# kaleo996/F5E-TTS

Hardware: AMD Instinct MI355X
Metric: mel_frames_per_sec (higher is better)
Workload: dtype bf16; 1 GPU; C2: F5TTS_v1_Base random-init, batch 1 per GPU, N_ref=188 N=469 frames, euler NFE=32, CFG=2.0 (cond+uncond batched), sway=-1.0, hipGraph ODE loop, HIP log-mel front-end + Vocos decode on GPU; parallelism=replica x1 (utterance sharding, no collective on the data path)

## Files before the change

### f5e-tts_amd/_C.py

```python
from __future__ import annotations

import ctypes as C
import os

_HERE = os.path.dirname(os.path.abspath(__file__))
LIB_PATH = os.environ.get("F5E_HIP_LIB") or os.path.join(_HERE, "libf5e_hip.so")

ABI_VERSION = 2

ACT_NONE, ACT_SILU, ACT_GELU_ERF, ACT_GELU_TANH, ACT_RELU, ACT_MISH = range(6)

_P, _I, _F, _LL = C.c_void_p, C.c_int, C.c_float, C.c_longlong

SIGNATURES = {
    "f5e_abi_version": [],
    "f5e_last_error": [],
    "f5e_check_device": [],
    "f5e_gemm_bf16_bias": [_P, _P, _I, _P, _I, _P, _P, _I, _I, _I, _I, _I, _I, _I],
    "f5e_gemm_bf16_gate_residual": [_P, _P, _I, _P, _I, _P, _P, _I, _P, _I, _I, _P, _I, _I, _P, _I, _I, _I, _I],
    "f5e_gemm_bf16_qkv_rope": [_P, _P, _I, _P, _I, _P, _P, _P, _P, _I, _I, _I, _P, _P, _P, _I, _I, _I, _I],
    "f5e_gemm_bf16_bias_ln": [_P, _P, _I, _P, _I, _P, _P, _I, _I, _I, _I, _I, _I, _I, _P],
    "f5e_gemm_bf16_gate_residual_ln": [_P, _P, _I, _P, _I, _P, _P, _I, _P, _I, _I, _P, _I, _I, _P, _I, _I, _I, _I, _P],
    "f5e_gemm_bf16_qkv_rope_ln": [_P, _P, _I, _P, _I, _P, _P, _P, _P, _I, _I, _I, _P, _P, _P, _I, _I, _I, _I, _P],
    "f5e_adaln_pre": [_P, _P, _I, _P, _I, _P, _I, _I, _I, _P, _I, _P, _I, _P, _I, _I],
    "f5e_flash_attn": [_P, _P, _P, _P, _P, _I, _P, _I, _I, _I, _I, _I],
    "f5e_joint_attn": [_P, _P, _P, _P, _P, _P, _P, _P, _I, _P, _I, _P, _I, _I, _I, _I, _I, _I, _I],
    "f5e_layernorm": [_P, _P, _I, _P, _I, _I, _P, _P, _P, _P, _I, _I, _I, _P, _I, _I, _I, _F],
    "f5e_grn": [_P, _P, _P, _P, _P, _P, _I, _I, _I],
    "f5e_l2norm": [_P, _P, _I, _P, _I, _I, _P, _I, _I],
    "f5e_gemm_f32": [_P, _P, _I, _I, _I, _P, _I, _P, _I, _P, _P, _I, _I, _P, _P, _I, _P, _I, _I, _I, _I],
    "f5e_convpos": [_P, _P, _I, _P, _P, _I, _P, _I, _P, _I, _P, _I, _I, _I, _I, _I],
    "f5e_dwconv7": [_P, _P, _P, _P, _P, _I, _I, _I],
    "f5e_im2col": [_P, _P, _P, _I, _I, _I, _I, _I],
    "f5e_sinus_embed": [_P, _P, _P, _P, _I, _I, _F],
    "f5e_rope_table": [_P, _P, _P, _I, _I],
    "f5e_text_gather": [_P, _P, _P, _P, _P, _P, _I, _I, _I, _I, _I],
    "f5e_ode_update": [_P, _P, _LL, _I, _F, _F, _P, _P, _P, _P, _P, _P, _LL],
    "f5e_ode_update_traj": [_P, _P, _LL, _I, _F, _F, _P, _P, _P, _LL, _I, _P, _P, _P, _LL],
    "f5e_advance_eval": [_P, _P],
    "f5e_stitch": [_P, _P, _P, _P, _P, _LL, _I],
    "f5e_cast_bf16": [_P, _P, _P, _LL],
    "f5e_cast_f32": [_P, _P, _P, _LL],
    "f5e_axpby": [_P, _P, _P, _P, _F, _F, _F, _LL],
    "f5e_vq_eval": [_P, _P, _I, _P, _I, _P, _P, _P, _I, _I, _I, _I],
    "f5e_mas_workspace_bytes": [_I, _I, _I, C.POINTER(C.c_ulonglong)],
    "f5e_mas_path": [_P, _P, _LL, _I, _P, _P, _P, _P, _P, C.c_ulonglong, _I, _I, _I],
    "f5e_resample": [_P, _P, _LL, _P, _I, _I, _I, _P, _LL, _I, _I, _I],
    "f5e_ctc_align_workspace_bytes": [_I, _I, _I, C.POINTER(C.c_ulonglong)],
    "f5e_ctc_align": [_P, _P, _LL, _I, _P, _I, _P, _P, _I, _P, _P, _P, _P, _P, C.c_ulonglong, _I, _I, _I, _I],
    "f5e_ctc_greedy": [_P, _P, _LL, _I, _P, _I, _I, _P, _P, _P, _I, _I, _I],
    "f5e_ctc_beam_workspace_bytes": [_I, _I, _I, C.POINTER(C.c_ulonglong)],
    "f5e_ctc_beam": [_P, _P, _LL, _I, _P, _I, _I, _P, _I, _P, _P, _P, C.c_ulonglong, _I, _I, _I],
    "f5e_token_logp": [_P, _P, _LL, _P, _P, _LL, _I],
    "f5e_log_softmax_rows": [_P, _P, _LL, _P, _LL, _LL, _I],
    "f5e_stft_logmel": [_P, _P, _I, _I, _P, _P, _P, _P, _I, _I, _I, _I],
    "f5e_stft_logmel_banded": [_P, _P, _I, _I, _P, _P, _P, _P, _I, _P, _I, _I, _I, _I],
    "f5e_stft_logmel_banded_ex": [_P, _P, _I, _I, _P, _P, _P, _P, _I, _P, _I, _I, _I, _I, _I, _I, _F],
    "f5e_bigvgan_act": [_P, _P, _P, _I, _P, _P, _P, _P, _I, _I, _I],
    "f5e_bigvgan_conv": [_P, _P, _P, _P, _P, _P, _P, _F, _I, _I, _I, _I, _I, _I, _I, _I, _I],
    "f5e_bigvgan_post": [_P, _P, _P, _P, _P, _I, _I, _I, _I, _I],
    "f5e_istft_head": [_P, _P, _I, _P, _P, _P, _P, _I, _I, _I, _I],
    "f5e_kaldi_fbank": [_P, _P, _I, _I, _P, _P, _P, _P, _I, _I, _I, _I, _F, _F, _F],
    "f5e_glu": [_P, _P, _I, _P, _I, _LL, _I],
    "f5e_dwconv": [_P, _P, _P, _P, _P, _P, _I, _I, _I, _I],
    "f5e_softmax_rows": [_P, _P, _I, _P, _I, _P, _LL, _I, _I, _F],
    "f5e_dwconv_stream": [_P, _P, _P, _P, _P, _P, _I, _I, _I, _I, _I, _I],
    "f5e_relpos_attn": [_P, _P, _I, _P, _I, _P, _I, _P, _I, _P, _I, _P, _I, _I, _I, _I, _I, _I, _I, _F],
    "f5e_mha_f32": [_P, _P, _I, _P, _I, _P, _I, _P, _I, _P, _I, _I, _I, _I, _I, _I, _F],
    "f5e_attn_decode_f32": [_P, _P, _I, _P, _P, _LL, _I, _P, _I, _P, _I, _I, _I, _I, _I, _I, _F],
    "f5e_beam_step": [_P, _P, _LL, _P, _P, _P, _P, _P, _I, _P, _P, _P, _I, _I, _I, _I, _I],
    "f5e_dit_forward": [_P, _P],
    "f5e_sample_loop": [_P, _P],
    "f5e_workspace_bytes": [_P, _P],
    "f5e_timer_create": [_I, C.POINTER(C.c_void_p)],
    "f5e_timer_destroy": [_P],
    "f5e_timer_reset": [_P],
    "f5e_timer_read": [_P, C.POINTER(C.c_float), _I, C.POINTER(C.c_int)],
    "f5e_timer_read_ops": [_P, C.POINTER(C.c_int), _I, C.POINTER(C.c_int)],
    "f5e_graph_begin": [_P],
    "f5e_graph_end": [_P, C.POINTER(C.c_void_p)],
    "f5e_graph_launch": [_P, _P],
    "f5e_graph_destroy": [_P],
}
_RESTYPE = {"f5e_last_error": C.c_char_p}
# ... 76 lines not shown
```

### f5e-tts_amd/csrc/conv.hip

```cpp
#include <cstdlib>
#include "f5e_common.h"

namespace {

struct ConvPosArgs {
  const bf16* x; int ldx;
  const bf16* w;
  const float* bias;
  bf16* out_bf16; int ldo;
  float* out_f32; int ldo32;
  const float* resid; int ldr;
  int S, N, D, mode, tiles_t, cpg;
  unsigned long long* trace;
};

__device__ __forceinline__ void glds16c(const void* g, void* lds) {
  __builtin_amdgcn_global_load_lds((const __attribute__((address_space(1))) void*)g,
                                   (__attribute__((address_space(3))) void*)lds, 16, 0, 0);
}

__device__ const uint4 conv_zero16 = {0u, 0u, 0u, 0u};

__device__ __forceinline__ void wait_vm_lgkm0(int n) {
  switch (n) {
// ... 253 lines not shown
      for (int i = 0; i < 4; ++i)
#pragma unroll
        for (int j = 0; j < 4; ++j)
          acc[i][j] = __builtin_amdgcn_mfma_f32_16x16x32_bf16(wf[i], xf[j], acc[i][j], 0, 0, 0);
    };
    if (live) reads(0);
    if (u + NST - 1 < 8) stage_w((u + NST - 1) % NST, u + NST - 1);
    if (!live) break;
    mfmas();
    reads(1);
    mfmas();
  }

  if constexpr (TRC) ts[5] = __builtin_amdgcn_s_memtime();
  asm volatile("s_waitcnt vmcnt(0) lgkmcnt(0)" ::: "memory");
  __builtin_amdgcn_s_barrier();
  float* mine = Red + wave * (64 * RS);
#pragma unroll
  for (int i = 0; i < 4; ++i)
#pragma unroll
    for (int j = 0; j < 4; ++j) *(f32x4*)(mine + (j * 16 + fr) * RS + i * 16 + fq * 4) = acc[i][j];
  asm volatile("s_waitcnt lgkmcnt(0)" ::: "memory");
  __builtin_amdgcn_s_barrier();
#pragma unroll
  for (int p = 0; p < 4; ++p) asm volatile("" : "+v"(rv[p]));

  if (oc < a.cpg) {
#pragma unroll
    for (int p = 0; p < 4; ++p) {
      const int row = wave * 16 + p * 4 + (lane >> 4);
      const int t = t0 + row;
      const size_t m = (size_t)seq * a.N + t;
      const float* rp = Red + row * RS + oc;
      f32x4 v = (*(const f32x4*)rp + *(const f32x4*)(rp + 64 * RS)) + (*(const f32x4*)(rp + 2 * 64 * RS) + *(const f32x4*)(rp + 3 * 64 * RS));
      v += bias;
      v[0] = mish_f(v[0]); v[1] = mish_f(v[1]); v[2] = mish_f(v[2]); v[3] = mish_f(v[3]);
      if (t >= a.N) continue;
      if (a.mode == 0) {
        *(bf16x4*)(a.out_bf16 + m * a.ldo + n) = f2bf4(v[0], v[1], v[2], v[3]);
      } else {
        v += rv[p];
        *(f32x4*)(a.out_f32 + m * a.ldo32 + n) = v;
      }
    }
  }
  if constexpr (TRC) {
    asm volatile("s_waitcnt vmcnt(0)" ::: "memory");
    ts[6] = __builtin_amdgcn_s_memtime(); ts[7] = __builtin_amdgcn_s_memrealtime();
    if (tid == 0 && a.trace) {
      unsigned long long* o = a.trace + ((size_t)(blockIdx.z * gridDim.y + blockIdx.y) * gridDim.x + blockIdx.x) * 8;
#pragma unroll
      for (int i = 0; i < 8; ++i) o[i] = ts[i];
    }
  }
}

__global__ __launch_bounds__(256) void dwconv7_kernel(const float* x, const float* wT, const float* bias, float* y,
                                                       int B, int T, int C) {
  const int c4n = C / 4;
  const size_t total = (size_t)B * T * c4n;
  for (size_t i = (size_t)blockIdx.x * 256 + threadIdx.x; i < total; i += (size_t)gridDim.x * 256) {
    const int c = (int)(i % c4n) * 4;
    const size_t bt = i / c4n;
    const int t = (int)(bt % T);
    const size_t b = bt / T;
    f32x4 acc = *(const f32x4*)(bias + c);
#pragma unroll
    for (int j = 0; j < 7; ++j) {
      const int tj = t + j - 3;
      if (tj >= 0 && tj < T)
        acc += *(const f32x4*)(wT + (size_t)j * C + c) * *(const f32x4*)(x + (b * T + tj) * C + c);
    }
    *(f32x4*)(y + (b * T + t) * C + c) = acc;
  }
}

__global__ __launch_bounds__(256) void im2col_kernel(const float* x, float* col, int B, int T, int Cin, int ksize,
                                                      int pad) {
  const size_t total = (size_t)B * T * ksize * Cin;
  for (size_t i = (size_t)blockIdx.x * 256 + threadIdx.x; i < total; i += (size_t)gridDim.x * 256) {
    const int ic = (int)(i % Cin);
    size_t r = i / Cin;
    const int j = (int)(r % ksize);
    r /= ksize;
    const int t = (int)(r % T);
    const size_t b = r / T;
    const int tj = t + j - pad;
    col[i] = (tj >= 0 && tj < T) ? x[(b * T + tj) * Cin + ic] : 0.f;
  }
}

inline int grid_for(size_t total) {
  size_t g = (total + 255) / 256;
  return (int)(g < 4096 ? (g ? g : 1) : 4096);
}

}

#ifdef F5E_TOOLS
static unsigned long long* g_convpos_trace = nullptr;
#define F5E_CONVPOS_TRACE g_convpos_trace
#else
#define F5E_CONVPOS_TRACE ((unsigned long long*)nullptr)
#endif

extern "C" {
// ... 8 lines not shown
  F5E_REQUIRE(x && w_packed && bias, "convpos: null operand");
  F5E_REQUIRE(S > 0 && N > 0 && D > 0 && groups > 0 && D % groups == 0, "convpos: bad D=%d / groups=%d", D, groups);
  const int cpg = D / groups;
  F5E_REQUIRE(cpg % 16 == 0 && cpg <= 64, "convpos: channels per group = %d must be 16, 32, 48 or 64", cpg);
  F5E_REQUIRE(ldx % 8 == 0, "convpos: ldx must be a multiple of 8");
  if (mode == 0) F5E_REQUIRE(out_bf16 && ldo % 4 == 0, "convpos: mode 0 needs a bf16 output");
  else {
    F5E_REQUIRE(mode == 1, "convpos: mode must be 0 or 1");
    F5E_REQUIRE(out_f32 && resid && ldo32 % 4 == 0 && ldr % 4 == 0, "convpos: mode 1 needs f32 output + residual");
  }
  ConvPosArgs a{};
  a.x = (const bf16*)x; a.ldx = ldx; a.w = (const bf16*)w_packed; a.bias = bias;
  a.out_bf16 = (bf16*)out_bf16; a.ldo = ldo; a.out_f32 = out_f32; a.ldo32 = ldo32; a.resid = resid; a.ldr = ldr;
  a.S = S; a.N = N; a.D = D; a.mode = mode; a.cpg = cpg;
  a.tiles_t = (N + 63) / 64;
  F5E_REQUIRE(a.tiles_t <= 65535 && S <= 65535, "convpos: grid too large");
  const dim3 grid(groups, a.tiles_t, S);
  const int xs = 96 * 128;
#ifdef F5E_TOOLS
  static const int forced = getenv("F5E_CONVPOS") ? atoi(getenv("F5E_CONVPOS")) : 0;
#else
  constexpr int forced = 0;
#endif
  const int n_cu = f5e_cu_count();
  const bool split = forced ? forced == 1 : (size_t)groups * a.tiles_t * S <= (size_t)n_cu;
  const int lds_split = xs + 4 * 4 * 8192, lds_ring = xs + 4 * 8192;
  a.trace = F5E_CONVPOS_TRACE;
  static F5eDeviceOnce once_split;
  if (split) F5E_OPT_IN_LDS(once_split, convpos_split_kernel<false>, lds_split);
#ifdef F5E_TOOLS
  static F5eDeviceOnce once_split_trace;
  if (split && a.trace) {
    F5E_OPT_IN_LDS(once_split_trace, convpos_split_kernel<true>, lds_split);
    hipLaunchKernelGGL(convpos_split_kernel<true>, grid, dim3(256), lds_split, st, a);
  } else if (a.trace) {
    hipLaunchKernelGGL((convpos_kernel<4, true>), grid, dim3(256), lds_ring, st, a);
  } else
#endif
  if (split) {
    hipLaunchKernelGGL(convpos_split_kernel<false>, grid, dim3(256), lds_split, st, a);
  } else {
    hipLaunchKernelGGL((convpos_kernel<4, false>), grid, dim3(256), lds_ring, st, a);
  }
  F5E_LAUNCH_CHECK("convpos");
  return F5E_OK;
}

int f5e_convpos(hipStream_t st, const void* x, int ldx, const void* w_packed, const float* bias, int mode,
                void* out_bf16, int ldo, float* out_f32, int ldo32, const float* resid, int ldr, int S, int N, int D,
                int groups) {
  return convpos_launch(st, x, ldx, w_packed, bias, mode, out_bf16, ldo, out_f32, ldo32, resid, ldr, S, N, D, groups);
}

int f5e_dwconv7(hipStream_t st, const float* x, const float* w_t, const float* bias, float* y, int B, int T, int C) {
  F5E_REQUIRE(x && w_t && bias && y, "dwconv7: null operand");
  F5E_REQUIRE(B > 0 && T > 0 && C > 0 && C % 4 == 0, "dwconv7: C=%d must be a positive multiple of 4", C);
  hipLaunchKernelGGL(dwconv7_kernel, dim3(grid_for((size_t)B * T * C / 4)), dim3(256), 0, st, x, w_t, bias, y, B, T, C);
  F5E_LAUNCH_CHECK("dwconv7");
  return F5E_OK;
}

int f5e_im2col(hipStream_t st, const float* x, float* col, int B, int T, int Cin, int ksize, int pad) {
  F5E_REQUIRE(x && col && B > 0 && T > 0 && Cin > 0 && ksize > 0 && pad >= 0, "im2col: bad arguments");
  hipLaunchKernelGGL(im2col_kernel, dim3(grid_for((size_t)B * T * Cin * ksize)), dim3(256), 0, st, x, col, B, T, Cin,
                     ksize, pad);
  F5E_LAUNCH_CHECK("im2col");
  return F5E_OK;
}

}
```

### f5e-tts_amd/csrc/runtime.hip

```cpp
#include <stdarg.h>
#include <stdio.h>
#include <string.h>
#include <cstdlib>

#include "f5e_common.h"
#include "gemm_bf16_args.h"

static thread_local char g_err[512] = "";

void f5e_set_error(const char* fmt, ...) {
  va_list ap;
  va_start(ap, fmt);
  vsnprintf(g_err, sizeof(g_err), fmt, ap);
  va_end(ap);
}

#define HIP_TRY(call, what)                                                        \
  do {                                                                             \
    hipError_t e_ = (call);                                                        \
    if (e_ != hipSuccess) {                                                        \
      f5e_set_error("%s: %s", what, hipGetErrorString(e_));                        \
      return F5E_ERR_HIP;                                                          \
    }                                                                              \
  } while (0)
// ... 113 lines not shown

int f5e_timer_reset(void* timer) {
  F5E_REQUIRE(timer, "timer_reset: null");
  ((F5eTimer*)timer)->count = 0;
  return F5E_OK;
}

int f5e_timer_read(void* timer, float* ms_out_host, int max_out, int* count_out_host) {
  F5E_REQUIRE(timer && ms_out_host && count_out_host, "timer_read: null");
  F5eTimer* t = (F5eTimer*)timer;
  const int n = t->count < max_out ? t->count : max_out;
  for (int i = 0; i < n; ++i) {
    HIP_TRY(hipEventSynchronize(t->stop[i]), "hipEventSynchronize");
    HIP_TRY(hipEventElapsedTime(&ms_out_host[i], t->start[i], t->stop[i]), "hipEventElapsedTime");
  }
  *count_out_host = n;
  return F5E_OK;
}

int f5e_timer_read_ops(void* timer, int* ops_out_host, int max_out, int* count_out_host) {
  F5E_REQUIRE(timer && ops_out_host && count_out_host, "timer_read_ops: null");
  F5eTimer* t = (F5eTimer*)timer;
  const int n = t->count < max_out ? t->count : max_out;
  for (int i = 0; i < n; ++i) ops_out_host[i] = t->op[i];
  *count_out_host = n;
  return F5E_OK;
}

#define F5E_TIMED(opclass, call)                                                  \
  do {                                                                            \
    const bool sel_ = p->timer_op >= 0 ? p->timer_op == (opclass) : (((-p->timer_op) >> (opclass)) & 1) != 0; \
    F5eTimer* tm_ = (p->timer && sel_) ? (F5eTimer*)p->timer : nullptr;          \
    const bool on_ = tm_ && tm_->count < tm_->capacity;                           \
    if (on_) HIP_TRY(hipEventRecord(tm_->start[tm_->count], st), "hipEventRecord"); \
    F5E_TRY(call);                                                                \
    if (on_) {                                                                    \
      HIP_TRY(hipEventRecord(tm_->stop[tm_->count], st), "hipEventRecord");       \
      tm_->op[tm_->count] = (opclass);                                            \
      tm_->count++;                                                               \
    }                                                                             \
  } while (0)

int f5e_dit_forward(hipStream_t st, const f5e_dit_plan* p) {
  F5E_REQUIRE(p, "dit_forward: null plan");
  F5E_REQUIRE(p->S > 0 && p->B > 0 && p->S % p->B == 0 && p->N > 0 && p->L > 0, "dit_forward: bad S/B/N/L");
  F5E_REQUIRE(p->D % 256 == 0 && p->H > 0 && p->FF % 64 == 0 && p->mel % 4 == 0, "dit_forward: unsupported dims");
  F5E_REQUIRE(p->y && p->w_x && p->in_const && p->rope_cs && p->mod && p->blocks && p->w_proj, "dit_forward: null input");
  F5E_REQUIRE(p->h0 && p->h0_bf16 && p->c1 && p->x && p->hn && p->q && p->k && p->vt && p->ao && p->ff && p->pred,
              "dit_forward: null workspace");
  const int M = p->S * p->N, D = p->D, inner = p->H * 64;
  const int row_stride = p->L * 6 * D + 2 * D;
  const int eval_stride = p->mod_rows * row_stride;

  F5E_TIMED(F5E_OP_INPROJ, f5e_gemm_f32(st, p->y, p->mel, p->B * p->N, F5E_ACT_NONE, p->w_x, p->ldw_x, nullptr, F5E_ACT_NONE, nullptr,
                       p->in_const, D, M, nullptr, p->h0, D, p->h0_bf16, D, M, D, p->mel));
  F5E_TIMED(F5E_OP_CONVPOS, f5e_convpos(st, p->h0_bf16, D, p->convpos_w1, p->convpos_b1, 0, p->c1, D, nullptr, 0, nullptr, 0, p->S, p->N, D, p->convpos_groups));
  F5E_TIMED(F5E_OP_CONVPOS, f5e_convpos(st, p->c1, D, p->convpos_w2, p->convpos_b2, 1, nullptr, 0, p->x, D, p->h0, D, p->S, p->N, D, p->convpos_groups));

  if (p->w_skip) {
    F5E_REQUIRE(p->skip_res && p->skip_tmp, "dit_forward: long skip needs skip_res / skip_tmp");
    HIP_TRY(hipMemcpyAsync(p->skip_res, p->x, (size_t)M * D * sizeof(float), hipMemcpyDeviceToDevice, st),
            "hipMemcpyAsync(skip_res)");
  }
  if (p->fuse_ln) {
    F5E_REQUIRE(!p->w_skip, "dit_forward: fused AdaLN does not cover the long skip connection");
    F5E_REQUIRE(p->ln_stats && p->ln_rowmean && p->cd && D % 256 == 0 && D <= 1024 && p->mod_rows == 1 && inner == D && p->cd_stride % 4 == 0,
                "dit_forward: fused AdaLN needs ln_stats, ln_rowmean, cd tables, D %% 256 == 0, D <= 1024, one modulation row and heads * 64 == D");
    const int parts = D / 64, ls = 6 * inner + 2 * p->FF, cd_eval_stride = p->mod_rows * p->cd_stride;
    F5E_REQUIRE(p->cd_stride >= p->L * ls + 2 * p->mel, "dit_forward: cd_stride too small");
    f5e_ln_fuse cons{}, prod{};
    cons.stats = p->ln_stats; cons.parts = parts; cons.cd_stride = p->cd_stride; cons.cd_rows = p->mod_rows;
    cons.cd_eval_stride = cd_eval_stride; cons.eval_ptr = p->eval_ptr; cons.rows_per_seq = p->N; cons.eps = 1e-6f;
    prod.xs_out = p->hn; prod.ld_xs = D; prod.stats_out = p->ln_stats;
    cons.row_mean = prod.row_mean = p->ln_rowmean;
    F5E_TIMED(F5E_OP_LN, f5e_adaln_pre(st, p->x, D, p->hn, D, p->mod + D, row_stride, p->mod_rows, p->N, p->eval_ptr, eval_stride,
                                       p->ln_stats, parts, p->ln_rowmean, M, D));
    const bool pfon = p->mall_prefetch != 0;
    const unsigned b_out = (unsigned)((size_t)D * inner * 2), b_ff = (unsigned)((size_t)p->FF * D * 2);
    const unsigned b_qkv = (unsigned)((size_t)3 * inner * D * 2);
    for (int l = 0; l < p->L; ++l) {
      const f5e_dit_block_weights& w = p->blocks[l];
      F5E_REQUIRE(!w.q_norm_w, "dit_forward: fused AdaLN and qk_norm are exclusive");
      const float* mb = p->mod + (size_t)l * 6 * D;
      const float* cdl = p->cd + (size_t)l * ls;
      const F5ePrefetch pf_next{{l + 1 < p->L ? p->blocks[l + 1].w_qkv : p->w_proj, nullptr},
                                {l + 1 < p->L ? b_qkv : (unsigned)((size_t)p->mel * D * 2), 0}};
      F5ePrefetch pf_qkv{{w.w_out, nullptr}, {b_out, 0}};
      F5ePrefetch pf_attn{{w.w_ff1, nullptr}, {b_ff, 0}};
      F5ePrefetch pf_out{{w.w_ff2, nullptr}, {b_ff, 0}};
      F5ePrefetch pf_nx = pf_next, pf_ff1{};
      {
        int scheme = 0;
#ifdef F5E_TOOLS
        static const int scheme_env = getenv("F5E_PF_SCHEME") ? atoi(getenv("F5E_PF_SCHEME")) : -1;
        if (scheme_env >= 0) scheme = scheme_env;
#endif
        const void* wout_next = l + 1 < p->L ? (const void*)p->blocks[l + 1].w_out : nullptr;
        if (scheme == 1 || scheme == 3) {
          pf_attn = F5ePrefetch{{w.w_ff1, w.w_ff2}, {b_ff, b_ff}};
          pf_out = F5ePrefetch{};
        }
        if (scheme == 2 || scheme == 3) {
          pf_nx = F5ePrefetch{{pf_next.ptr[0], wout_next}, {pf_next.bytes[0], wout_next ? b_out : 0}};
          if (l > 0) pf_qkv = F5ePrefetch{};
        }
#ifdef F5E_TOOLS
        if (scheme == 5 || scheme == 6) {
          pf_qkv = F5ePrefetch{{w.w_out, w.w_ff1}, {b_out, b_ff}};
          pf_attn = F5ePrefetch{};
          if (scheme == 6) { pf_out = F5ePrefetch{}; pf_ff1 = F5ePrefetch{{w.w_ff2, nullptr}, {b_ff, 0}}; }
// ... 92 lines not shown
```

### f5e-tts_amd/ops.py

```python
from __future__ import annotations

import ctypes as C
import threading
from typing import Optional

import torch

from . import _C
from ._C import ACT_GELU_ERF, ACT_GELU_TANH, ACT_MISH, ACT_NONE, ACT_RELU, ACT_SILU, check, lib

Tensor = torch.Tensor
_checked_device = False


def _stream() -> int:
    return torch.cuda.current_stream().cuda_stream


def require_device() -> None:
    global _checked_device
    if not _checked_device:
        if not torch.cuda.is_available():
            raise _C.F5EError("f5e_tts_amd needs a ROCm GPU (gfx950); torch.cuda.is_available() is False and there "
                              "is no CPU fallback")
# ... 200 lines not shown

def grn(x: Tensor, out: Tensor, gamma: Tensor, beta: Tensor, ws: Tensor):
    require_device()
    B, T, Cc = x.shape
    check(lib().f5e_grn(_stream(), _p(x, F32, "x"), _p(out, F32, "out"), _p(ws, F32, "ws"), _p(gamma, F32, "gamma"),
                        _p(beta, F32, "beta"), B, T, Cc), "f5e_grn")
    return out


def gemm_f32(a: Tensor, w: Tensor, bias: Optional[Tensor] = None, *, out: Optional[Tensor] = None,
             out_bf16: Optional[Tensor] = None, M: Optional[int] = None, a_act: int = ACT_NONE, act: int = ACT_NONE,
             ch_scale: Optional[Tensor] = None, addend: Optional[Tensor] = None, row_scale: Optional[Tensor] = None,
             K: Optional[int] = None):
    require_device()
    a_rows = a.shape[0]
    K = a.shape[1] if K is None else K
    N = w.shape[0]
    M = a_rows if M is None else M
    for t, nm in ((a, "a"), (w, "w")):
        if not t.is_cuda or t.dtype != F32 or t.stride(1) != 1:
            raise _C.F5EError(f"gemm_f32: {nm} must be an f32 GPU tensor with unit column stride")
    ad = addend
    check(lib().f5e_gemm_f32(
        _stream(), C.c_void_p(a.data_ptr()), a.stride(0), a_rows, a_act, C.c_void_p(w.data_ptr()), w.stride(0),
        _p(bias, F32, "bias"), act, _p(ch_scale, F32, "ch_scale"),
        C.c_void_p(ad.data_ptr()) if ad is not None else None, ad.stride(0) if ad is not None else 0,
        ad.shape[0] if ad is not None else 0, _p(row_scale, F32, "row_scale"),
        C.c_void_p(out.data_ptr()) if out is not None else None, out.stride(0) if out is not None else 0,
        C.c_void_p(out_bf16.data_ptr()) if out_bf16 is not None else None,
        out_bf16.stride(0) if out_bf16 is not None else 0, M, N, K), "f5e_gemm_f32")
    return out if out is not None else out_bf16


def pack_convpos_weight(w: Tensor, groups: int = 16) -> Tensor:
    D, cpg, taps = w.shape
    out = torch.zeros(groups, taps, 64, 64, dtype=w.dtype, device=w.device)
    out[:, :, :cpg, :cpg] = w.view(groups, cpg, cpg, taps).permute(0, 3, 1, 2)
    return out.to(BF).contiguous()


def convpos(x: Tensor, w_packed: Tensor, bias: Tensor, S: int, N: int, *, out_bf16: Optional[Tensor] = None,
            out_f32: Optional[Tensor] = None, resid: Optional[Tensor] = None):
    require_device()
    D = x.shape[1]
    mode = 0 if out_f32 is None else 1
    check(lib().f5e_convpos(_stream(), _p(x, BF, "x"), x.stride(0), _p(w_packed, BF, "w_packed"), _p(bias, F32, "bias"),
                            mode, _p(out_bf16, BF, "out_bf16"), out_bf16.stride(0) if out_bf16 is not None else 0,
                            _p(out_f32, F32, "out_f32"), out_f32.stride(0) if out_f32 is not None else 0,
                            _p(resid, F32, "resid"), resid.stride(0) if resid is not None else 0, S, N, D,
                            w_packed.shape[0]),
          "f5e_convpos")


def dwconv7(x: Tensor, w_t: Tensor, bias: Tensor, out: Tensor):
    require_device()
    B, T, Cc = x.shape
    check(lib().f5e_dwconv7(_stream(), _p(x, F32, "x"), _p(w_t, F32, "w_t"), _p(bias, F32, "bias"), _p(out, F32, "out"),
                            B, T, Cc), "f5e_dwconv7")
    return out


def im2col(x: Tensor, col: Tensor, ksize: int, pad: int):
    require_device()
    B, T, Cin = x.shape
    check(lib().f5e_im2col(_stream(), _p(x, F32, "x"), _p(col, F32, "col"), B, T, Cin, ksize, pad), "f5e_im2col")
    return col


def sinus_embed(t: Tensor, freqs: Tensor, out: Tensor, scale: float = 1000.0):
    require_device()
    E, dim = out.shape
    check(lib().f5e_sinus_embed(_stream(), _p(t, F32, "t"), _p(freqs, F32, "freqs"), _p(out, F32, "out"), E, dim, scale),
          "f5e_sinus_embed")
    return out


def rope_table(inv_freq: Tensor, out: Tensor):
    require_device()
    N, half, _ = out.shape
    check(lib().f5e_rope_table(_stream(), _p(inv_freq, F32, "inv_freq"), _p(out, F32, "out"), N, half), "f5e_rope_table")
    return out


def text_gather(ids: Tensor, table: Tensor, pos: Optional[Tensor], keep: Optional[Tensor], out: Tensor):
    require_device()
    B, N, TD = out.shape
    check(lib().f5e_text_gather(_stream(), _p(ids, I32, "ids"), _p(table, F32, "table"), _p(pos, F32, "pos"),
                                _p(keep, F32, "keep"), _p(out, F32, "out"), B, N, TD,
                                pos.shape[0] if pos is not None else 1, table.shape[0]), "f5e_text_gather")
    return out


def ode_update(pred: Tensor, branch_stride: int, mode: int, w0: float, w1: float, base: Tensor, dst: Tensor,
               coef: Tensor, eval_ptr: Optional[Tensor], traj: Optional[Tensor] = None,
               done_ctr: Optional[Tensor] = None, traj_stride: int = 0, traj_div: int = 1):
    require_device()
    check(lib().f5e_ode_update_traj(_stream(), _p(pred, F32, "pred"), branch_stride, mode, w0, w1, _p(base, F32, "base"),
                                    _p(dst, F32, "dst"), C.c_void_p(traj.data_ptr()) if traj is not None else None,
                                    traj_stride, traj_div, _p(coef, F32, "coef"), _p(eval_ptr, I32, "eval_ptr"),
                                    _p(done_ctr, I32, "done_ctr"), base.numel()), "f5e_ode_update")
    return dst


def sample_loop(loop: "_C.LoopPlan"):
    require_device()
    check(lib().f5e_sample_loop(_stream(), C.byref(loop)), "f5e_sample_loop")
# ... 562 lines not shown
```

### include/f5e_abi.h

```cpp
#ifndef F5E_ABI_H_
#define F5E_ABI_H_

#ifdef __cplusplus
extern "C" {
#endif

#define F5E_ABI_VERSION 2

#if defined(__GNUC__)
#define F5E_API __attribute__((visibility("default")))
#else
#define F5E_API
#endif

enum { F5E_OK = 0, F5E_ERR_BAD_SHAPE = -1, F5E_ERR_UNSUPPORTED = -2, F5E_ERR_HIP = -3 };

enum { F5E_ACT_NONE = 0, F5E_ACT_SILU = 1, F5E_ACT_GELU_ERF = 2, F5E_ACT_GELU_TANH = 3, F5E_ACT_RELU = 4, F5E_ACT_MISH = 5 };

#ifdef F5E_STREAM_T
typedef F5E_STREAM_T f5e_stream;
#else
typedef void* f5e_stream;
#endif

// ... 16 lines not shown
                           int tile_hint);

typedef struct f5e_ln_fuse {
  const float* stats; int parts;
  const float* c; const float* d; int cd_stride; int cd_rows; int cd_eval_stride;
  const int* eval_ptr; int rows_per_seq; float eps;
  void* xs_out; int ld_xs; const float* next_scale;
  float* stats_out;
  float* row_mean;
} f5e_ln_fuse;

F5E_API int f5e_gemm_bf16_bias_ln(f5e_stream st, const void* A, int lda, const void* W, int ldw, const float* bias, void* out,
                          int ldo, int M, int N, int K, int act, int out_f32, int tile_hint, const f5e_ln_fuse* ln);
F5E_API int f5e_gemm_bf16_gate_residual_ln(f5e_stream st, const void* A, int lda, const void* W, int ldw, const float* bias,
                                   float* resid, int ldr, const float* gate, int gate_stride, int gate_rows,
                                   const int* eval_ptr, int eval_stride, int rows_per_seq, const int* seq_len, int M,
                                   int N, int K, int tile_hint, const f5e_ln_fuse* ln);
F5E_API int f5e_gemm_bf16_qkv_rope_ln(f5e_stream st, const void* A, int lda, const void* W, int ldw, const float* bias,
                              void* q, void* k, void* vt, int n_pad, int heads, int rope_heads, const float* cos_sin,
                              const float* q_norm_w, const float* k_norm_w, int rows_per_seq, int M, int K,
                              int tile_hint, const f5e_ln_fuse* ln);


F5E_API int f5e_flash_attn(f5e_stream st, const void* q, const void* k, const void* vt, void* o, int ldo, const int* kv_len,
                   int S, int H, int rows_per_seq, int n_pad, int splits);

F5E_API int f5e_joint_attn(f5e_stream st, const void* qx, const void* kx, const void* vx, const void* qc, const void* kc,
                   const void* vc, void* o_x, int ldo_x, void* o_c, int ldo_c, const int* kv_len, int S, int H, int N,
                   int n_pad_x, int Nt, int n_pad_c, int splits);


F5E_API int f5e_layernorm(f5e_stream st, const float* x, int ldx, void* y, int ldy, int y_bf16, const float* gamma,
                  const float* beta, const float* scale, const float* shift, int mod_stride, int mod_rows,
                  int rows_per_seq, const int* eval_ptr, int eval_stride, int rows, int D, float eps);

F5E_API int f5e_adaln_pre(f5e_stream st, const float* x, int ldx, void* xs, int ld_xs, const float* scale, int mod_stride,
                  int mod_rows, int rows_per_seq, const int* eval_ptr, int eval_stride, float* stats, int parts,
                  float* row_mean, int rows, int D);

F5E_API int f5e_l2norm(f5e_stream st, const float* x, int ldx, void* y, int ldy, int y_bf16, const float* g, int rows, int D);

F5E_API int f5e_grn(f5e_stream st, const float* x, float* y, float* gx_ws, const float* gamma, const float* beta, int B, int T,
            int C);


F5E_API int f5e_gemm_f32(f5e_stream st, const float* A, int lda, int a_rows, int a_act, const float* W, int ldw,
                 const float* bias, int act, const float* ch_scale, const float* addend, int ld_add, int add_rows,
                 const float* row_scale, float* out, int ldo, void* out_bf16, int ldo_bf16, int M, int N, int K);


F5E_API int f5e_convpos(f5e_stream st, const void* x, int ldx, const void* w_packed, const float* bias, int mode,
                void* out_bf16, int ldo, float* out_f32, int ldo32, const float* resid, int ldr, int S, int N, int D,
                int groups);

F5E_API int f5e_dwconv7(f5e_stream st, const float* x, const float* w_t, const float* bias, float* y, int B, int T, int C);

F5E_API int f5e_im2col(f5e_stream st, const float* x, float* col, int B, int T, int Cin, int ksize, int pad);


F5E_API int f5e_sinus_embed(f5e_stream st, const float* t, const float* freqs, float* out, int E, int dim, float scale);
F5E_API int f5e_rope_table(f5e_stream st, const float* inv_freq, float* out, int N, int half);
F5E_API int f5e_text_gather(f5e_stream st, const int* ids, const float* table, const float* pos, const float* keep, float* out,
                    int B, int N, int TD, int max_pos, int table_rows);
F5E_API int f5e_ode_update(f5e_stream st, const float* pred, long long branch_stride, int mode, float w0, float w1,
                   const float* base, float* dst, float* traj, const float* coef, int* eval_ptr, unsigned* done_ctr,
                   long long n);
F5E_API int f5e_ode_update_traj(f5e_stream st, const float* pred, long long branch_stride, int mode, float w0, float w1,
                        const float* base, float* dst, float* traj, long long traj_stride, int traj_div,
                        const float* coef, int* eval_ptr, unsigned* done_ctr, long long n);
F5E_API int f5e_advance_eval(f5e_stream st, int* eval_ptr);
F5E_API int f5e_stitch(f5e_stream st, const float* cond, const float* y, const unsigned char* mask, float* out, long long rows,
               int C);
F5E_API int f5e_cast_bf16(f5e_stream st, const float* x, void* y, long long n);
F5E_API int f5e_cast_f32(f5e_stream st, const void* x, float* y, long long n);
F5E_API int f5e_axpby(f5e_stream st, const float* x, const float* y, float* out, float a, float b, float c, long long n);
F5E_API int f5e_vq_eval(f5e_stream st, const float* logits, int ld, const float* vars, int combine_groups, float* out,
                int* targets, float* stats, int rows, int groups, int num_vars, int var_dim);

F5E_API int f5e_mas_workspace_bytes(int B, int Ty, int Tx, unsigned long long* bytes_out_host);
F5E_API int f5e_mas_path(f5e_stream st, const float* logp, long long batch_stride, int ld, const int* t_y, const int* t_x,
                 int* token_of_frame, int* durations, void* workspace, unsigned long long workspace_bytes, int B, int Ty,
                 int Tx);

F5E_API int f5e_resample(f5e_stream st, const float* x, long long ld_x, const float* bank, int orig, int new_, int width,
                 float* y, long long ld_y, int B, int n, int n_out);

F5E_API int f5e_ctc_align_workspace_bytes(int B, int T, int L, unsigned long long* bytes_out_host);
F5E_API int f5e_ctc_align(f5e_stream st, const float* scores, long long batch_stride, int ld, const int* labels, int ld_labels,
                  const int* t_len, const int* l_len, int blank, int* align, int* tok_start, int* tok_end, float* score,
                  void* workspace, unsigned long long workspace_bytes, int B, int T, int L, int V);

F5E_API int f5e_ctc_greedy(f5e_stream st, const float* scores, long long batch_stride, int ld, const int* t_len, int blank,
                   int pad_id, int* hyp, int* hyp_len, float* frame_logp, int B, int T, int V);

F5E_API int f5e_ctc_beam_workspace_bytes(int B, int T, int beam, unsigned long long* bytes_out_host);
F5E_API int f5e_ctc_beam(f5e_stream st, const float* scores, long long batch_stride, int ld, const int* t_len, int blank,
                 int beam, int* hyp, int ld_hyp, int* hyp_len, float* score, void* workspace,
                 unsigned long long workspace_bytes, int B, int T, int V);

F5E_API int f5e_token_logp(f5e_stream st, const float* logits, long long ld, const int* target, float* out, long long rows,
                   int V);
F5E_API int f5e_log_softmax_rows(f5e_stream st, const float* x, long long ldx, float* out, long long ldo, long long rows,
                         int V);


F5E_API int f5e_stft_logmel(f5e_stream st, const float* wav, int nw, int ldw, const float* window, const float* twiddle,
// ... 137 lines not shown
```

Before: 12980 mel-frames/s.

## Fuse input projection and both conv-position layers into one kernel

Adds a single kernel that computes the mel input projection with fp32 MFMA, keeps the result in LDS as bf16, and then runs both grouped 31-tap conv-position layers with split-tap accumulation across waves and the residual add. This removes two kernel launches and the global round trips of h0 and the intermediate conv output in each DiT evaluation. In exchange, each time tile recomputes halo rows, and the path is used only when the whole grid fits within the CU count and the layout constraints hold.

Result: no change. 13030 mel-frames/s, median of 6 (+0.4%).

```diff
diff --git a/f5e-tts_amd/_C.py b/f5e-tts_amd/_C.py
--- a/f5e-tts_amd/_C.py
+++ b/f5e-tts_amd/_C.py
@@ -30,6 +30,7 @@
     "f5e_l2norm": [_P, _P, _I, _P, _I, _I, _P, _I, _I],
     "f5e_gemm_f32": [_P, _P, _I, _I, _I, _P, _I, _P, _I, _P, _P, _I, _I, _P, _P, _I, _P, _I, _I, _I, _I],
     "f5e_convpos": [_P, _P, _I, _P, _P, _I, _P, _I, _P, _I, _P, _I, _I, _I, _I, _I],
+    "f5e_embed_convpos": [_P, _P, _I, _I, _P, _I, _I, _P, _I, _P, _P, _P, _P, _P, _I, _I, _I, _I, _I],
     "f5e_dwconv7": [_P, _P, _P, _P, _P, _I, _I, _I],
     "f5e_im2col": [_P, _P, _P, _I, _I, _I, _I, _I],
     "f5e_sinus_embed": [_P, _P, _P, _P, _I, _I, _F],
diff --git a/f5e-tts_amd/csrc/conv.hip b/f5e-tts_amd/csrc/conv.hip
--- a/f5e-tts_amd/csrc/conv.hip
+++ b/f5e-tts_amd/csrc/conv.hip
@@ -329,6 +329,261 @@
 #pragma unroll
       for (int i = 0; i < 8; ++i) o[i] = ts[i];
     }
+  }
+}
+
+struct EmbedConvArgs {
+  const float* y; int ldy; int y_rows;
+  const float* wx; int ldw; int K;
+  const float* addc; int ld_add;
+  const bf16* w1; const float* b1;
+  const bf16* w2; const float* b2;
+  float* out; int ldo;
+  int S, N, D;
+};
+
+struct TapRing {
+  const bf16* w_src[8];
+  char* ring;
+  int wave;
+  __device__ __forceinline__ void init(const bf16* wg, char* ring_base, int wave_, int lane) {
+    wave = wave_;
+    ring = ring_base + wave_ * (4 * 8192);
+#pragma unroll
+    for (int j = 0; j < 8; ++j) {
+      const int i = lane + 64 * j;
+      const int row = i >> 3, c = (i & 7) ^ ((row >> 1) & 7);
+      w_src[j] = wg + row * 64 + c * 8;
+    }
+  }
+  __device__ __forceinline__ void stage(int slot, int u) const {
+    int tap = wave + 4 * u;
+    tap = tap < 31 ? tap : 30;
+#pragma unroll
+    for (int j = 0; j < 8; ++j) glds16c(w_src[j] + (size_t)tap * 4096, ring + slot * 8192 + j * 1024);
+  }
+};
+
+template <int RT, int ROT>
+__device__ __forceinline__ void split_tap_loop(const char* Xs, const TapRing& rg, int lane, f32x4 (&acc)[4][RT]) {
+  constexpr int W_BYTES = 8192, NST = 4, TAPS = 31;
+  const int fr = lane & 15, fq = lane >> 4;
+#pragma unroll
+  for (int i = 0; i < 4; ++i)
+#pragma unroll
+    for (int j = 0; j < RT; ++j) acc[i][j] = f32x4{0.f, 0.f, 0.f, 0.f};
+#pragma unroll
+  for (int u = 0; u < 8; ++u) {
+    const int issued = u + NST - 1 < 8 ? u + NST - 1 : 8;
+    const int pend = 8 * (issued - u - 1);
+    if (pend == 16) asm volatile("s_waitcnt vmcnt(16) lgkmcnt(0)" ::: "memory");
+    else if (pend == 8) asm volatile("s_waitcnt vmcnt(8) lgkmcnt(0)" ::: "memory");
+    else asm volatile("s_waitcnt vmcnt(0) lgkmcnt(0)" ::: "memory");
+    if (u == 0) __builtin_amdgcn_s_barrier();
+    const int tap = rg.wave + 4 * u;
+    const bool live = !(u == 7 && tap >= TAPS);
+    const char* Ws = rg.ring + ((u + ROT) % NST) * W_BYTES;
+    bf16x8 xf[RT], wf[4];
+    auto reads = [&](int kk) {
+      const int c = kk * 4 + fq;
+#pragma unroll
+      for (int j = 0; j < RT; ++j) {
+        const int row = j * 16 + fr + tap;
+        xf[j] = *(const bf16x8*)(Xs + row * 128 + ((c ^ ((row >> 1) & 7)) << 4));
+      }
+#pragma unroll
+      for (int i = 0; i < 4; ++i) {
+        const int row = i * 16 + fr;
+        wf[i] = *(const bf16x8*)(Ws + row * 128 + ((c ^ ((row >> 1) & 7)) << 4));
+      }
+    };
+    auto mfmas = [&]() {
+#pragma unroll
+      for (int i = 0; i < 4; ++i)
+#pragma unroll
+        for (int j = 0; j < RT; ++j)
+          acc[i][j] = __builtin_amdgcn_mfma_f32_16x16x32_bf16(wf[i], xf[j], acc[i][j], 0, 0, 0);
+    };
+    if (live) reads(0);
+    if (u + NST - 1 < 8) rg.stage((u + NST - 1 + ROT) % NST, u + NST - 1);
+    if (!live) break;
+    mfmas();
+    reads(1);
+    mfmas();
+  }
+}
+
+__device__ __forceinline__ int red_off(int row, int q) { return row * 256 + ((q ^ (row & 15)) << 4); }
+
+template <int RT>
+__device__ __forceinline__ void split_tap_partials(char* my_ring, int lane, const f32x4 (&acc)[4][RT]) {
+  const int fr = lane & 15, fq = lane >> 4;
+#pragma unroll
+  for (int i = 0; i < 4; ++i)
+#pragma unroll
+    for (int j = 0; j < RT; ++j) *(f32x4*)(my_ring + red_off(j * 16 + fr, i * 4 + fq)) = acc[i][j];
+}
+__device__ __forceinline__ f32x4 split_tap_sum(const char* ring_base, int row, int q) {
+  const char* rp = ring_base + red_off(row, q);
+  return (*(const f32x4*)rp + *(const f32x4*)(rp + 32768)) + (*(const f32x4*)(rp + 2 * 32768) + *(const f32x4*)(rp + 3 * 32768));
+}
+
+__global__ __launch_bounds__(256) void embed_convpos_kernel(EmbedConvArgs a) {
+  constexpr int BT = 64, HALO = 15;
+  constexpr int T0_BYTES = 128 * 128, R0_BYTES = 64 * 256;
+  extern __shared__ __attribute__((aligned(16))) char smem[];
+  char* T0 = smem;
+  char* R0 = smem + T0_BYTES;
+  char* ring_base = smem + T0_BYTES + R0_BYTES;
+
+  const int tid = threadIdx.x, lane = tid & 63;
+  const int wave = __builtin_amdgcn_readfirstlane(tid >> 6);
+  const int g = blockIdx.x, tt = blockIdx.y, seq = blockIdx.z;
+  const int c0 = g * 64;
+  const int t0 = tt * BT;
+  const int fr = lane & 15, fq = lane >> 4;
+  const int oc = fr * 4;
+
+  f32x4 xf[2][4][2], add[4][2];
+  bool valid[2];
+#pragma unroll
+  for (int j = 0; j < 2; ++j) {
+    const int t = t0 - 2 * HALO + wave * 32 + j * 16 + fr;
+    valid[j] = t >= 0 && t < a.N;
+    const size_t m = (size_t)seq * a.N + (t < 0 ? 0 : (t < a.N ? t : a.N - 1));
+    const float* ap = a.y + (m % (size_t)a.y_rows) * a.ldy;
+#pragma unroll
+    for (int kt = 0; kt < 2; ++kt)
+#pragma unroll
+      for (int s = 0; s < 4; ++s) {
+        const int k0 = kt * 64 + s * 16 + fq * 4;
+        xf[kt][s][j] = k0 < a.K ? *(const f32x4*)(ap + k0) : f32x4{0.f, 0.f, 0.f, 0.f};
+      }
+    const float* cp = a.addc + m * a.ld_add + c0 + fq * 4;
+#pragma unroll
+    for (int i = 0; i < 4; ++i) add[i][j] = *(const f32x4*)(cp + i * 16);
+  }
+  f32x4 bias1 = *(const f32x4*)(a.b1 + c0 + oc);
+  f32x4 bias2 = *(const f32x4*)(a.b2 + c0 + oc);
+  asm volatile("" ::: "memory");
+  __builtin_amdgcn_sched_barrier(0);
+#pragma unroll
+  for (int q = 0; q < 8; ++q) {
+    const int i = lane + 64 * q;
+    const int row = wave * 16 + (i >> 5), c = (i & 31) ^ (row & 15);
+    const void* src = &conv_zero16;
+    if (c * 4 < a.K) src = a.wx + (size_t)(c0 + row) * a.ldw + c * 4;
+    glds16c(src, ring_base + wave * (4 * 8192) + 3 * 8192 + q * 1024);
+  }
+  asm volatile("s_waitcnt vmcnt(0)" ::: "memory");
+#pragma unroll
+  for (int j = 0; j < 2; ++j) {
+#pragma unroll
+    for (int i = 0; i < 4; ++i) asm volatile("" : "+v"(add[i][j]));
+#pragma unroll
+    for (int kt = 0; kt < 2; ++kt)
+#pragma unroll
+      for (int s = 0; s < 4; ++s) asm volatile("" : "+v"(xf[kt][s][j]));
+  }
+  asm volatile("" : "+v"(bias1));
+  asm volatile("" : "+v"(bias2));
+  __builtin_amdgcn_s_barrier();
+  TapRing rg;
+  rg.init(a.w1 + (size_t)g * 31 * 4096, ring_base, wave, lane);
+#pragma unroll
+  for (int u = 0; u < 3; ++u) rg.stage(u, u);
+  asm volatile("" ::: "memory");
+  __builtin_amdgcn_sched_barrier(0);
+
+  {
+    f32x4 acc[4][2];
+#pragma unroll
+    for (int i = 0; i < 4; ++i)
+#pragma unroll
+      for (int j = 0; j < 2; ++j) acc[i][j] = f32x4{0.f, 0.f, 0.f, 0.f};
+#pragma unroll
+    for (int kt = 0; kt < 2; ++kt) {
+      if (kt * 64 < a.K) {
+#pragma unroll
+        for (int s = 0; s < 4; ++s) {
+          if (kt * 64 + s * 16 >= a.K) break;
+          f32x4 wf[4];
+#pragma unroll
+          for (int i = 0; i < 4; ++i) {
+            const int row = i * 16 + fr, c = (kt * 16 + s * 4 + fq) ^ (row & 15);
+            wf[i] = *(const f32x4*)(ring_base + (row >> 4) * (4 * 8192) + 3 * 8192 + (row & 15) * 512 + (c << 4));
+          }
+#pragma unroll
+          for (int r = 0; r < 4; ++r)
+#pragma unroll
+            for (int i = 0; i < 4; ++i)
+#pragma unroll
+              for (int j = 0; j < 2; ++j)
+                acc[i][j] = __builtin_amdgcn_mfma_f32_16x16x4f32(wf[i][r], xf[kt][s][j][r], acc[i][j], 0, 0, 0);
+        }
+      }
+    }
+#pragma unroll
+    for (int j = 0; j < 2; ++j) {
+      const int row = wave * 32 + j * 16 + fr;
+      const int cr = row - 2 * HALO;
+#pragma unroll
+      for (int i = 0; i < 4; ++i) {
+        const f32x4 v = acc[i][j] + add[i][j];
+        bf16x4 b = f2bf4(v[0], v[1], v[2], v[3]);
+        if (!valid[j]) b = f2bf4(0.f, 0.f, 0.f, 0.f);
+        const int c = i * 2 + (fq >> 1);
+        *(bf16x4*)(T0 + row * 128 + ((c ^ ((row >> 1) & 7)) << 4) + (fq & 1) * 8) = b;
+        if (cr >= 0 && cr < BT) *(f32x4*)(R0 + cr * 256 + (((i * 4 + fq) ^ (cr & 15)) << 4)) = v;
+      }
+    }
+  }
+
+  {
+    f32x4 acc[4][6];
+    split_tap_loop<6, 0>(T0, rg, lane, acc);
+    asm volatile("s_waitcnt vmcnt(0) lgkmcnt(0)" ::: "memory");
+    rg.init(a.w2 + (size_t)g * 31 * 4096, ring_base, wave, lane);
+    rg.stage(3, 0);
+    split_tap_partials<6>(rg.ring, lane, acc);
+  }
+  asm volatile("s_waitcnt lgkmcnt(0)" ::: "memory");
+  __builtin_amdgcn_s_barrier();
+#pragma unroll
+  for (int p = 0; p < 6; ++p) {
+    const int row = wave * 24 + p * 4 + fq;
+    const int t = t0 - HALO + row;
+    f32x4 v = split_tap_sum(ring_base, row, fr);
+    v += bias1;
+    v[0] = mish_f(v[0]); v[1] = mish_f(v[1]); v[2] = mish_f(v[2]); v[3] = mish_f(v[3]);
+    bf16x4 b = f2bf4(v[0], v[1], v[2], v[3]);
+    if (t < 0 || t >= a.N) b = f2bf4(0.f, 0.f, 0.f, 0.f);
+    const int c = fr >> 1;
+    *(bf16x4*)(T0 + row * 128 + ((c ^ ((row >> 1) & 7)) << 4) + (fr & 1) * 8) = b;
+  }
+  asm volatile("s_waitcnt lgkmcnt(0)" ::: "memory");
+  __builtin_amdgcn_s_barrier();
+
+  rg.stage(0, 1);
+  rg.stage(1, 2);
+  {
+    f32x4 acc[4][4];
+    split_tap_loop<4, 3>(T0, rg, lane, acc);
+    asm volatile("s_waitcnt vmcnt(0) lgkmcnt(0)" ::: "memory");
+    split_tap_partials<4>(rg.ring, lane, acc);
+  }
+  asm volatile("s_waitcnt lgkmcnt(0)" ::: "memory");
+  __builtin_amdgcn_s_barrier();
+#pragma unroll
+  for (int p = 0; p < 4; ++p) {
+    const int row = wave * 16 + p * 4 + fq;
+    const int t = t0 + row;
+    f32x4 v = split_tap_sum(ring_base, row, fr);
+    v += bias2;
+    v[0] = mish_f(v[0]); v[1] = mish_f(v[1]); v[2] = mish_f(v[2]); v[3] = mish_f(v[3]);
+    if (t >= a.N) continue;
+    v += *(const f32x4*)(R0 + row * 256 + ((fr ^ (row & 15)) << 4));
+    *(f32x4*)(a.out + ((size_t)seq * a.N + t) * a.ldo + c0 + oc) = v;
   }
 }
 
@@ -443,6 +698,31 @@
   return convpos_launch(st, x, ldx, w_packed, bias, mode, out_bf16, ldo, out_f32, ldo32, resid, ldr, S, N, D, groups);
 }
 
+int f5e_embed_convpos(hipStream_t st, const float* y, int ldy, int y_rows, const float* w_x, int ldw_x, int K,
+                      const float* in_const, int ld_const, const void* w1_packed, const float* b1, const void* w2_packed,
+                      const float* b2, float* x_out, int ldo, int S, int N, int D, int groups) {
+  F5E_REQUIRE(y && w_x && in_const && w1_packed && b1 && w2_packed && b2 && x_out, "embed_convpos: null operand");
+  F5E_REQUIRE(S > 0 && N > 0 && D > 0 && groups > 0 && y_rows > 0, "embed_convpos: bad S=%d N=%d D=%d groups=%d", S, N, D, groups);
+  F5E_REQUIRE(D == groups * 64, "embed_convpos: channels per group must be 64 (D=%d, groups=%d)", D, groups);
+  F5E_REQUIRE(K > 0 && K % 4 == 0 && K <= 128, "embed_convpos: K=%d must be a multiple of 4, at most 128", K);
+  F5E_REQUIRE(ldy % 4 == 0 && ldy >= K && ldw_x % 4 == 0 && ldw_x >= K && ld_const % 4 == 0 && ld_const >= D && ldo % 4 == 0 && ldo >= D,
+              "embed_convpos: leading dimensions must be multiples of 4 that cover their rows");
+  F5E_REQUIRE((((uintptr_t)y | (uintptr_t)w_x | (uintptr_t)in_const | (uintptr_t)b1 | (uintptr_t)b2 | (uintptr_t)x_out |
+                (uintptr_t)w1_packed | (uintptr_t)w2_packed) & 15) == 0, "embed_convpos: operands must be 16-byte aligned");
+  EmbedConvArgs a{};
+  a.y = y; a.ldy = ldy; a.y_rows = y_rows; a.wx = w_x; a.ldw = ldw_x; a.K = K; a.addc = in_const; a.ld_add = ld_const;
+  a.w1 = (const bf16*)w1_packed; a.b1 = b1; a.w2 = (const bf16*)w2_packed; a.b2 = b2; a.out = x_out; a.ldo = ldo;
+  a.S = S; a.N = N; a.D = D;
+  const int tiles_t = (N + 63) / 64;
+  F5E_REQUIRE(tiles_t <= 65535 && S <= 65535, "embed_convpos: grid too large");
+  constexpr int lds = 128 * 128 + 64 * 256 + 4 * 4 * 8192;
+  static F5eDeviceOnce once;
+  F5E_OPT_IN_LDS(once, embed_convpos_kernel, lds);
+  hipLaunchKernelGGL(embed_convpos_kernel, dim3(groups, tiles_t, S), dim3(256), lds, st, a);
+  F5E_LAUNCH_CHECK("embed_convpos");
+  return F5E_OK;
+}
+
 int f5e_dwconv7(hipStream_t st, const float* x, const float* w_t, const float* bias, float* y, int B, int T, int C) {
   F5E_REQUIRE(x && w_t && bias && y, "dwconv7: null operand");
   F5E_REQUIRE(B > 0 && T > 0 && C > 0 && C % 4 == 0, "dwconv7: C=%d must be a positive multiple of 4", C);
diff --git a/f5e-tts_amd/csrc/runtime.hip b/f5e-tts_amd/csrc/runtime.hip
--- a/f5e-tts_amd/csrc/runtime.hip
+++ b/f5e-tts_amd/csrc/runtime.hip
@@ -189,10 +189,20 @@
   const int row_stride = p->L * 6 * D + 2 * D;
   const int eval_stride = p->mod_rows * row_stride;
 
-  F5E_TIMED(F5E_OP_INPROJ, f5e_gemm_f32(st, p->y, p->mel, p->B * p->N, F5E_ACT_NONE, p->w_x, p->ldw_x, nullptr, F5E_ACT_NONE, nullptr,
-                       p->in_const, D, M, nullptr, p->h0, D, p->h0_bf16, D, M, D, p->mel));
-  F5E_TIMED(F5E_OP_CONVPOS, f5e_convpos(st, p->h0_bf16, D, p->convpos_w1, p->convpos_b1, 0, p->c1, D, nullptr, 0, nullptr, 0, p->S, p->N, D, p->convpos_groups));
-  F5E_TIMED(F5E_OP_CONVPOS, f5e_convpos(st, p->c1, D, p->convpos_w2, p->convpos_b2, 1, nullptr, 0, p->x, D, p->h0, D, p->S, p->N, D, p->convpos_groups));
+  const bool head_fused = p->convpos_groups > 0 && D == p->convpos_groups * 64 && !p->w_skip && p->mel <= 128 && p->ldw_x % 4 == 0 &&
+                          (((uintptr_t)p->y | (uintptr_t)p->w_x | (uintptr_t)p->in_const | (uintptr_t)p->x | (uintptr_t)p->convpos_w1 |
+                            (uintptr_t)p->convpos_b1 | (uintptr_t)p->convpos_w2 | (uintptr_t)p->convpos_b2) & 15) == 0 &&
+                          (size_t)((p->N + 63) / 64) * p->convpos_groups * p->S <= (size_t)f5e_cu_count();
+  if (head_fused) {
+    F5E_TIMED(F5E_OP_CONVPOS, f5e_embed_convpos(st, p->y, p->mel, p->B * p->N, p->w_x, p->ldw_x, p->mel, p->in_const, D,
+                                                p->convpos_w1, p->convpos_b1, p->convpos_w2, p->convpos_b2, p->x, D, p->S,
+                                                p->N, D, p->convpos_groups));
+  } else {
+    F5E_TIMED(F5E_OP_INPROJ, f5e_gemm_f32(st, p->y, p->mel, p->B * p->N, F5E_ACT_NONE, p->w_x, p->ldw_x, nullptr, F5E_ACT_NONE, nullptr,
+                         p->in_const, D, M, nullptr, p->h0, D, p->h0_bf16, D, M, D, p->mel));
+    F5E_TIMED(F5E_OP_CONVPOS, f5e_convpos(st, p->h0_bf16, D, p->convpos_w1, p->convpos_b1, 0, p->c1, D, nullptr, 0, nullptr, 0, p->S, p->N, D, p->convpos_groups));
+    F5E_TIMED(F5E_OP_CONVPOS, f5e_convpos(st, p->c1, D, p->convpos_w2, p->convpos_b2, 1, nullptr, 0, p->x, D, p->h0, D, p->S, p->N, D, p->convpos_groups));
+  }
 
   if (p->w_skip) {
     F5E_REQUIRE(p->skip_res && p->skip_tmp, "dit_forward: long skip needs skip_res / skip_tmp");
diff --git a/f5e-tts_amd/ops.py b/f5e-tts_amd/ops.py
--- a/f5e-tts_amd/ops.py
+++ b/f5e-tts_amd/ops.py
@@ -276,6 +276,20 @@
           "f5e_convpos")
 
 
+def embed_convpos(y: Tensor, w_x: Tensor, in_const: Tensor, w1_packed: Tensor, b1: Tensor, w2_packed: Tensor, b2: Tensor,
+                  S: int, N: int, out: Tensor):
+    require_device()
+    D, K = w_x.shape[0], y.shape[1]
+    (yp, ldy), (wp, ldw) = _rows(y, (F32,), "y", K), _rows(w_x, (F32,), "w_x", K)
+    (cp, ldc), (op, ldo) = _rows(in_const, (F32,), "in_const", D), _rows(out, (F32,), "out", D)
+    if in_const.shape[0] != S * N or out.shape[0] != S * N or (S * N) % y.shape[0]:
+        raise _C.F5EError(f"embed_convpos: in_const and out need S * N = {S * N} rows, y a divisor of that")
+    check(lib().f5e_embed_convpos(_stream(), yp, ldy, y.shape[0], wp, ldw, K, cp, ldc, _p(w1_packed, BF, "w1_packed"),
+                                  _p(b1, F32, "b1"), _p(w2_packed, BF, "w2_packed"), _p(b2, F32, "b2"), op, ldo, S, N, D,
+                                  w1_packed.shape[0]), "f5e_embed_convpos")
+    return out
+
+
 def dwconv7(x: Tensor, w_t: Tensor, bias: Tensor, out: Tensor):
     require_device()
     B, T, Cc = x.shape
diff --git a/include/f5e_abi.h b/include/f5e_abi.h
--- a/include/f5e_abi.h
+++ b/include/f5e_abi.h
@@ -92,6 +92,10 @@
 F5E_API int f5e_convpos(f5e_stream st, const void* x, int ldx, const void* w_packed, const float* bias, int mode,
                 void* out_bf16, int ldo, float* out_f32, int ldo32, const float* resid, int ldr, int S, int N, int D,
                 int groups);
+
+F5E_API int f5e_embed_convpos(f5e_stream st, const float* y, int ldy, int y_rows, const float* w_x, int ldw_x, int K,
+                      const float* in_const, int ld_const, const void* w1_packed, const float* b1, const void* w2_packed,
+                      const float* b2, float* x_out, int ldo, int S, int N, int D, int groups);
 
 F5E_API int f5e_dwconv7(f5e_stream st, const float* x, const float* w_t, const float* bias, float* y, int B, int T, int C);
 
```
